# grantjr1842/delayed-streams-modeling

Hardware: AMD Instinct MI355X
Metric: real-time stream throughput, stt-1b-en_fr @ bs=64 per GPU (Mimi encode + LM decode per 80 ms frame) (higher is better)
Workload: dtype bf16 weights + bf16 KV, f32 activations as three exact bf16 pieces, f32 accumulate (v_mfma_f32_16x16x32_bf16); 1 GPU; stt-1b-en_fr batch=64 streaming, ring KV cache full (750 frames), Mimi encode + LM decode HIP path; streams_per_gpu=64, parallelism=replicas x1 (independent stream batches, no per-step collective), streams=encoder stream || 2 LM group stream(s)

## Files before the change

delayed-streams-modeling_amd/csrc/dsm_engine.hip:

```cpp
#include <hip/hip_runtime.h>

#include <cmath>
#include <cstdarg>
#include <cstdio>
#include <cstdlib>
#include <cstring>
#include <atomic>
#include <mutex>
#include <shared_mutex>
#include <string>
#include <set>
#include <vector>

#include "../../include/dsm.h"
#include "dsm_config_presets.h"
#include "dsm_kernels.h"
#include "dsm_numerics.h"
#include "dsm_safetensors.h"

static thread_local std::string g_create_error;

#define HIPCHK_E(eng, expr)                                                                         \
  do {                                                                                              \
    hipError_t _e = (expr);                                                                         \
// ... 23 lines not shown
  bool replicate = false;
};

struct TLayerW {
  Linear in_proj, out_proj, ff_in, ff_out;
  float *n1w = nullptr, *n1b = nullptr, *n2w = nullptr, *n2b = nullptr, *ls1 = nullptr, *ls2 = nullptr;
  Linear ca_q, ca_kv, ca_out;
  float *ncw = nullptr, *ncb = nullptr;
};

struct TransformerW {
  dsm_transformer_config cfg{};
  int hidden = 0;
  std::vector<TLayerW> layers;
  float* inv_freq = nullptr;
  bool rope_pos_before = false;
  bool has_ca = false;
  int ca_norm_rms = 0;
};

struct CaState {
  std::vector<void*> k, v;
  uint32_t* last = nullptr;
  uint8_t* act = nullptr;
  float* att = nullptr;
  int smax = 0;
};

struct TransformerState {
  std::vector<void*> k, v;
  uint32_t *pos = nullptr, *idx = nullptr, *start_pos = nullptr, *widx = nullptr;
  float* rope_cs = nullptr;
};

struct RvqW {
  Linear input_proj, output_proj;
  int n_q = 0;
  std::vector<Linear> codebooks;
};

struct MimiW {
  dsm_mimi_config cfg{};
  ConvGeom init_conv, final_conv, downsample;
  struct Stage {
    ConvGeom ra, rb, down;
  };
  std::vector<Stage> stages;
  TransformerW tr;
  RvqW rvq_first, rvq_rest;
  struct DecStage {
    Linear up;
    float* up_bias = nullptr;
    int in_c = 0, out_c = 0, k = 0, stride = 0, T_in = 0;
    ConvGeom ra, rb;
  };
  bool has_decoder = false;
  ConvGeom dec_init, dec_final;
  std::vector<DecStage> dec_stages;
  TransformerW dec_tr;
  float* upsample_w = nullptr;
  const float** emb_ptrs = nullptr;
};

struct MimiState {
  float* pcm = nullptr;
  float* cat_init = nullptr;
  struct Stage {
    float *y = nullptr, *cat_ra = nullptr, *cat_rb = nullptr, *cat_down = nullptr;
  };
  std::vector<Stage> stages;
  float* cat_final = nullptr;
  float *x_tr = nullptr, *xn = nullptr, *q = nullptr, *att = nullptr, *ff = nullptr;
  float* cat_ds = nullptr;
  float* latent = nullptr;
  float *res_first = nullptr, *res_rest = nullptr, *pval = nullptr;
  uint32_t* pidx = nullptr;
  uint32_t* codes = nullptr;
  TransformerState tr;
  ConvStateDesc* descs = nullptr;
  std::vector<ConvStateDesc> h_descs;
  int ds_desc = -1;
  bool first_call = true;
  uint8_t* mask = nullptr;
};

struct MimiDecState {
  bool ready = false, first_call = true;
  uint32_t* codes = nullptr;
  uint8_t* mask = nullptr;
  uint8_t* started = nullptr;
  float *q_first = nullptr, *q_rest = nullptr, *emb = nullptr, *up_carry = nullptr;
  float *x_tr = nullptr, *xn = nullptr, *q = nullptr, *att = nullptr, *ff = nullptr;
  TransformerState tr;
  float* cat_init = nullptr;
  struct Stage {
    float *x = nullptr, *z = nullptr, *carry = nullptr, *y = nullptr, *cat_ra = nullptr, *cat_rb = nullptr;
  };
  std::vector<Stage> stages;
  float* cat_final = nullptr;
  float* pcm = nullptr;
  ConvStateDesc* descs = nullptr;
  std::vector<ConvStateDesc> h_descs;
};

struct LmW {
  uint16_t* text_emb = nullptr;
  uint16_t* audio_emb = nullptr;
  TransformerW tr;
  float* out_norm = nullptr;
  Linear text_linear, extra_heads;
};

struct LmState {
  float *x = nullptr, *xn = nullptr, *q = nullptr, *att = nullptr, *g = nullptr, *hidden = nullptr, *logits = nullptr,
        *eh = nullptr, *prs = nullptr;
  uint32_t *next_cb = nullptr, *text_token = nullptr, *text_out = nullptr, *codes_in = nullptr;
  uint8_t *first_step = nullptr, *mask = nullptr;
  uint32_t* rng_key = nullptr;
  unsigned long long* rng_pos = nullptr;
  uint8_t* gmask = nullptr;
  TransformerState tr;
  struct Group {
    int b0 = 0, nb = 0;
    TransformerState view;
  };
  std::vector<Group> groups;
};

struct HostItem {
  size_t step_idx = 0;
  std::vector<uint32_t> word_tokens;
  bool unended_word = false;
  double last_stop_time = 0.0;
};

}

struct dsm_engine {
  dsm_asr_config cfg{};
  int B = 0, device = 0;
  hipStream_t s_enc = nullptr, s_model = nullptr;
  static constexpr int kMaxGroups = 4;
  hipStream_t s_grp[kMaxGroups] = {nullptr, nullptr, nullptr, nullptr};
  hipEvent_t ev_fork = nullptr, ev_grp_in[kMaxGroups] = {}, ev_grp_done[kMaxGroups] = {}, ev_stagger[kMaxGroups] = {};
  bool grp_busy = false;
  bool use_graphs = true;
  bool fuse_qkv = true;
  bool stream_prio = false;
  bool fuse_front = false;
  int chunk_loop_min_tiles = 384;
  int loop_depth = 4;
  int smallk_min_tiles = 1024;
  int smallk_mt = 4;
  size_t attn_lds_pad = 60000;
  int dot_mode = 0;
  int prio_hi = 0;
  bool serialize_groups = false;
  hipEvent_t ev_codes_consumed = nullptr;
  bool codes_consumed_valid = false;
  hipEvent_t ev_join = nullptr, ev_a = nullptr, ev_b = nullptr, ev_c = nullptr, ev_d = nullptr;
  MimiW mimi_w;
  MimiState mimi[2];
  std::atomic<bool> mimi1_ready{false};
  std::mutex mimi1_mu;
  MimiDecState dec;
  float* h_pcm_out = nullptr;
  LmW lm_w;
  LmState lm;
  std::vector<void*> allocs;
  std::string err;
  float* h_pcm = nullptr;
  float* h_pcm1 = nullptr;
  uint8_t* h_mask = nullptr;
  uint32_t *h_codes = nullptr, *h_text = nullptr;
  float* h_prs = nullptr;
  std::vector<HostItem> items;
  size_t model_step_idx = 0;
  std::vector<dsm_asr_msg> msgs;
  std::vector<uint32_t> msg_tokens;
  dsm_metrics metrics{};
  static constexpr int kStreams = 1 + kMaxGroups;
  float* gemm_ws[kStreams] = {};
  size_t gemm_ws_cap[kStreams] = {};
  std::atomic<uint64_t> ws_gen{0};
  struct GraphSlot {
    hipGraphExec_t exec = nullptr;
    uint64_t key = 0, ws_gen = 0;
    int warm = 0;
    int failures = 0;
    bool disabled = false;
  };
  static constexpr int kMaxCaptureTries = 3;
  static thread_local bool capturing;
  bool capture_failed = false;
  GraphSlot g_enc[2], g_grp[kMaxGroups], g_dec, g_ttsg[kMaxGroups][2];
  std::atomic<uint64_t> graph_launches{0}, eager_bodies{0}, capture_failures{0};
  std::string capture_error;
  void note_capture_failure(const char* what, hipError_t he) {
    capture_failures += 1;
    std::lock_guard<std::mutex> lk(err_mu);
    if (capture_error.empty()) {
      capture_error = what;
      if (he != hipSuccess) { capture_error += ": "; capture_error += hipGetErrorString(he); }
    }
  }
  static constexpr int kPipe = 4;
  struct PipeSlot {
    float* h_pcm = nullptr;
    uint8_t* h_mask = nullptr;
    uint32_t* d_codes = nullptr;
    hipEvent_t ev_done = nullptr, ev_consumed = nullptr;
    bool in_flight = false;
  };
  PipeSlot pipe[kPipe];
  int pipe_next = 0;
  bool pipe_ready = false;
  std::mutex pipe_mu;
  std::shared_mutex api_mu;
  static thread_local std::shared_lock<std::shared_mutex>* api_held;
  unsigned prof_mask = 0;
  int tag_gemm[kStreams] = {DSM_PROF_OTHER, DSM_PROF_OTHER, DSM_PROF_OTHER, DSM_PROF_OTHER, DSM_PROF_OTHER};
  int tag_attn[kStreams] = {DSM_PROF_OTHER, DSM_PROF_OTHER, DSM_PROF_OTHER, DSM_PROF_OTHER, DSM_PROF_OTHER};
  std::mutex prof_mu, err_mu;
  int sid(hipStream_t st) const {
    if (st == s_enc) return 0;
    for (int g = 1; g < kMaxGroups; ++g)
      if (st == s_grp[g]) return 1 + g;
    return 1;
  }
  struct ProfRec {
    int tag;
    hipEvent_t a, b;
  };
  std::vector<ProfRec> prof_recs;
  std::vector<hipEvent_t> prof_pool;
  double prof_total_us[DSM_PROF_NTAGS] = {0};
  uint64_t prof_launches[DSM_PROF_NTAGS] = {0};

  static constexpr size_t kDevTsCap = 1 << 16;
  unsigned long long* dev_ts = nullptr;
  std::vector<int> dev_ts_tags;
  std::vector<int> dev_ts_info;
  bool timeline = false;
  unsigned long long* dev_ts_slot(int tag, int sid_ = 0, int kind = 0, int n = 1) {
    if (!dev_ts || !(prof_mask & (1u << tag))) return nullptr;
    std::lock_guard<std::mutex> lk(prof_mu);
    if (dev_ts_tags.size() + n > kDevTsCap) return nullptr;
    unsigned long long* p = dev_ts + 2 * dev_ts_tags.size();
    for (int i = 0; i < n; ++i) {
      dev_ts_tags.push_back(tag);
      dev_ts_info.push_back((sid_ << 8) | (kind + i));
    }
    return p;
  }

  hipEvent_t prof_event() {
    if (!prof_pool.empty()) {
      hipEvent_t ev = prof_pool.back();
      prof_pool.pop_back();
      return ev;
    }
    hipEvent_t ev = nullptr;
    (void)hipEventCreate(&ev);
    return ev;
  }
  int prof_begin(int tag, hipStream_t st) {
    if (!(prof_mask & (1u << tag))) return -1;
    std::lock_guard<std::mutex> lk(prof_mu);
    ProfRec r{tag, prof_event(), prof_event()};
    (void)hipEventRecord(r.a, st);
    prof_recs.push_back(r);
    return (int)prof_recs.size() - 1;
  }
  void prof_end(int h, hipStream_t st) {
    if (h < 0) return;
    std::lock_guard<std::mutex> lk(prof_mu);
    (void)hipEventRecord(prof_recs[h].b, st);
  }

  void set_error(const char* fmt, ...) {
    char buf[1024];
    va_list ap;
    va_start(ap, fmt);
    vsnprintf(buf, sizeof buf, fmt, ap);
    va_end(ap);
    std::lock_guard<std::mutex> lk(err_mu);
    err = buf;
  }

  template <typename T>
  int dalloc(T** out, size_t count, bool zero = true) {
    void* p = nullptr;
    size_t bytes = count * sizeof(T) + 256;
    HIPCHK_E(this, hipMalloc(&p, bytes));
    if (zero) {
      HIPCHK_E(this, hipMemset(p, 0, bytes));
      HIPCHK_E(this, hipStreamSynchronize(nullptr));
    }
    allocs.push_back(p);
    *out = reinterpret_cast<T*>(p);
    return 0;
  }
  template <typename T>
  int upload(T** out, const T* host, size_t count) {
    if (int rc = dalloc(out, count)) return rc;
    HIPCHK_E(this, hipMemcpy(*out, host, count * sizeof(T), hipMemcpyHostToDevice));
// ... 373 lines not shown
  if (cfg.quantizer_n_q > 1)
    if (int rc = load_rvq(e, ld, &m->rvq_rest, "quantizer.rvq_rest", cfg.quantizer_n_q - 1, cfg)) return rc;
  m->has_decoder = ld.has("decoder.model.0.conv.conv.weight") || ld.has("decoder.model.0.conv.conv.weight_v");
  if (!m->has_decoder) return 0;
  {
    int mult = 1 << cfg.n_ratios, idx = 0, T = m->final_conv.T_out;
    char p[128];
    snprintf(p, sizeof p, "decoder.model.%d", idx);
    if (int rc = load_conv(e, ld, &m->dec_init, p, cfg.dimension, mult * cfg.n_filters, cfg.kernel_size, 1, true, false)) return rc;
    m->dec_init.T_in = m->dec_init.T_out = T;
    idx += 1;
    m->dec_stages.resize(cfg.n_ratios);
    for (int i = 0; i < cfg.n_ratios; ++i) {
      const int ratio = cfg.ratios[i];
      MimiW::DecStage& st = m->dec_stages[i];
      st.in_c = mult * cfg.n_filters;
      st.out_c = st.in_c / 2;
      st.k = 2 * ratio;
      st.stride = ratio;
      st.T_in = T;
      snprintf(p, sizeof p, "decoder.model.%d.convtr.convtr", idx + 1);
      std::vector<float> w;
      if (ld.has("%s.weight", p)) {
        w = ld.get((int64_t)st.in_c * st.out_c * st.k, "%s.weight", p);
      } else {
        auto g = ld.get(st.in_c, "%s.weight_g", p);
        w = ld.get((int64_t)st.in_c * st.out_c * st.k, "%s.weight_v", p);
        for (int ci = 0; ci < st.in_c && !ld.failed; ++ci) {
          float ss = 0.0f;
          const size_t n = (size_t)st.out_c * st.k;
          for (size_t j = 0; j < n; ++j) ss = ss + w[ci * n + j] * w[ci * n + j];
          float nrm = sqrtf(ss);
          for (size_t j = 0; j < n; ++j) w[ci * n + j] = w[ci * n + j] * g[ci] / nrm;
        }
      }
      auto b = ld.get(st.out_c, "%s.bias", p);
      if (ld.failed) return DSM_ERR_IO;
      std::vector<float> r((size_t)st.k * st.out_c * st.in_c);
      for (int ci = 0; ci < st.in_c; ++ci)
        for (int co = 0; co < st.out_c; ++co)
          for (int kk = 0; kk < st.k; ++kk)
            r[((size_t)kk * st.out_c + co) * st.in_c + ci] = w[((size_t)ci * st.out_c + co) * st.k + kk];
      if (int rc = pack_linear(e, &st.up, r.data(), st.k * st.out_c, st.in_c, false, nullptr)) return rc;
      if (int rc = e->upload_w(&st.up_bias, b.data(), b.size())) return rc;
      idx += 2;
      T *= ratio;
      const int dim = st.out_c, hidden = dim / cfg.compress;
      snprintf(p, sizeof p, "decoder.model.%d.block.1", idx);
      if (int rc = load_conv(e, ld, &st.ra, p, dim, hidden, cfg.residual_kernel_size, 1, true, false)) return rc;
      snprintf(p, sizeof p, "decoder.model.%d.block.3", idx);
      if (int rc = load_conv(e, ld, &st.rb, p, hidden, dim, 1, 1, true, false)) return rc;
      st.ra.T_in = st.ra.T_out = st.rb.T_in = st.rb.T_out = T;
      idx += 1;
      mult /= 2;
    }
    snprintf(p, sizeof p, "decoder.model.%d", idx + 1);
    if (int rc = load_conv(e, ld, &m->dec_final, p, cfg.n_filters, cfg.channels, cfg.last_kernel_size, 1, true, false)) return rc;
    m->dec_final.T_in = m->dec_final.T_out = T;
    if (T != DSM_FRAME_SIZE) {
      e->set_error("decoder emits %d samples per step, expected %d", T, DSM_FRAME_SIZE);
      return DSM_ERR_INVALID;
    }
    if (int rc = load_transformer(e, ld, &m->dec_tr, cfg.transformer, "decoder_transformer.transformer", false)) return rc;
    const int st_ = cfg.downsample_stride, dim = cfg.dimension;
    auto uw = ld.get((int64_t)dim * 2 * st_, "upsample.convtr.convtr.convtr.weight");
    if (ld.failed) return DSM_ERR_IO;
    std::vector<float> ur((size_t)2 * st_ * dim);
    for (int c = 0; c < dim; ++c)
      for (int kk = 0; kk < 2 * st_; ++kk) ur[(size_t)kk * dim + c] = uw[(size_t)c * 2 * st_ + kk];
    if (int rc = e->upload_w(&m->upsample_w, ur.data(), ur.size())) return rc;
    std::vector<const float*> ptrs;
    ptrs.push_back(reinterpret_cast<const float*>(m->rvq_first.codebooks[0].w));
    for (auto& cb : m->rvq_rest.codebooks) ptrs.push_back(reinterpret_cast<const float*>(cb.w));
    if (e->wmode != dsm_engine::W_MEASURE)
      if (int rc = e->upload(&m->emb_ptrs, ptrs.data(), ptrs.size())) return rc;
  }
  return 0;
}

int alloc_cat(dsm_engine* e, float** out, const ConvGeom& c, int B) {
  return e->dalloc(out, (size_t)B * (c.S + c.T_in) * c.in_c);
}

void add_desc(MimiState* s, float* cat, const ConvGeom& c) {
  if (c.S == 0) return;
  ConvStateDesc d;
  d.cat = cat;
  d.bstride = (long)(c.S + c.T_in) * c.in_c;
  d.S = c.S;
  d.T = c.T_in;
  d.C = c.in_c;
  d.replicate = c.replicate ? 1 : 0;
  s->h_descs.push_back(d);
}

int alloc_mimi_state(dsm_engine* e, MimiState* s, const MimiW& w, int B) {
  const dsm_mimi_config& cfg = w.cfg;
  if (int rc = alloc_cat(e, &s->cat_init, w.init_conv, B)) return rc;
  add_desc(s, s->cat_init, w.init_conv);
  s->stages.resize(w.stages.size());
  for (size_t i = 0; i < w.stages.size(); ++i) {
    const MimiW::Stage& st = w.stages[i];
    if (int rc = e->dalloc(&s->stages[i].y, (size_t)B * st.ra.T_in * st.ra.in_c)) return rc;
    if (int rc = alloc_cat(e, &s->stages[i].cat_ra, st.ra, B)) return rc;
    if (int rc = alloc_cat(e, &s->stages[i].cat_rb, st.rb, B)) return rc;
    if (int rc = alloc_cat(e, &s->stages[i].cat_down, st.down, B)) return rc;
    add_desc(s, s->stages[i].cat_ra, st.ra);
    add_desc(s, s->stages[i].cat_rb, st.rb);
    add_desc(s, s->stages[i].cat_down, st.down);
  }
  if (int rc = alloc_cat(e, &s->cat_final, w.final_conv, B)) return rc;
  add_desc(s, s->cat_final, w.final_conv);
  const int Tt = w.final_conv.T_out, d = cfg.dimension;
  if (int rc = e->dalloc(&s->x_tr, (size_t)B * Tt * d)) return rc;
  if (int rc = e->dalloc(&s->xn, (size_t)B * Tt * d)) return rc;
  if (int rc = e->dalloc(&s->q, (size_t)B * Tt * d)) return rc;
  if (int rc = e->dalloc(&s->att, (size_t)B * Tt * d)) return rc;
  if (int rc = e->dalloc(&s->ff, (size_t)B * Tt * cfg.transformer.dim_feedforward)) return rc;
  if (int rc = alloc_cat(e, &s->cat_ds, w.downsample, B)) return rc;
  s->ds_desc = (int)s->h_descs.size();
  add_desc(s, s->cat_ds, w.downsample);
  if (int rc = e->dalloc(&s->latent, (size_t)B * d)) return rc;
  if (int rc = e->dalloc(&s->res_first, (size_t)B * cfg.quantizer_dim)) return rc;
  if (int rc = e->dalloc(&s->res_rest, (size_t)B * cfg.quantizer_dim)) return rc;
  const int n_tiles = (cfg.quantizer_bins + 15) / 16;
  if (int rc = e->dalloc(&s->pval, (size_t)n_tiles * B)) return rc;
  if (int rc = e->dalloc(&s->pidx, (size_t)n_tiles * B)) return rc;
  if (int rc = e->dalloc(&s->codes, (size_t)B * cfg.quantizer_n_q)) return rc;
  if (int rc = e->dalloc(&s->mask, B)) return rc;
  if (int rc = alloc_transformer_state(e, &s->tr, cfg.transformer, B, Tt, false)) return rc;
  if (int rc = e->upload(&s->descs, s->h_descs.data(), s->h_descs.size())) return rc;
  s->pcm = s->cat_init + (size_t)w.init_conv.S * w.init_conv.in_c;
  return 0;
}

bool wk_applicable(const dsm_engine* e, bool bf16_weights, int Kpad, int K, int M) {
  const int chunks = (Kpad + DSM_KC - 1) / DSM_KC;
  return bf16_weights && e->dot_mode == 1 && K % 32 == 0 && Kpad == K && chunks <= 4 && M <= 64;
}

template <typename WT, typename KVT, int EPI, int NT, int MT>
void launch_tile(hipStream_t st, dim3 grid, const GemmArgs& a, bool bx3, bool roll, bool deep) {
  constexpr int DMAX = LoopDepth<WT, NT>::MAX;
  if (bx3 && EPI != EPI_RVQ) {
    if (a.chunk_loop > 1) hipLaunchKernelGGL((gemm_bx3_kernel<KVT, MT, NT, EPI, true>), grid, dim3(256), 0, st, a);
    else if constexpr (MT == 4) hipLaunchKernelGGL((gemm_bx3_kernel<KVT, 4, NT, EPI, false>), grid, dim3(256), 0, st, a);
    else if constexpr (MT == 2) hipLaunchKernelGGL((gemm_bx3u_kernel<KVT, 2, NT, EPI, 8, 0, 4>), grid, dim3(256), 8 * 3 * 32 * 32 * 2, st, a);
    else hipLaunchKernelGGL((gemm_bx3u_kernel<KVT, 1, NT, EPI, 8>), grid, dim3(256), 8 * 3 * 16 * 32 * 2, st, a);
  } else if (roll && deep) hipLaunchKernelGGL((gemm_loop_kernel<WT, KVT, MT, NT, EPI, DMAX>), grid, dim3(256), 0, st, a);
  else if (roll) hipLaunchKernelGGL((gemm_loop_kernel<WT, KVT, MT, NT, EPI, 2>), grid, dim3(256), 0, st, a);
  else hipLaunchKernelGGL((gemm_tile_kernel<WT, KVT, MT, NT, EPI>), grid, dim3(256), 0, st, a);
}

template <typename WT, typename KVT, int EPI, int NT>
int launch_gemm_tiled(dsm_engine* e, hipStream_t st, GemmArgs& a) {
  int chunks = (a.Kpad + DSM_KC - 1) / DSM_KC;
  const int gx = (a.N + 63) / 64;
  const bool bx3 = e->dot_mode == 1 && sizeof(WT) == 2;
  auto ok4 = [](const RowMap& m) { return m.ld % 4 == 0 && m.bstride % 4 == 0; };
  a.vec = (a.N % 4 == 0) && (!a.Y || ok4(a.ymap)) && (!a.Y2 || ok4(a.y2map)) && (!a.res || ok4(a.rmap));
  a.chunk_loop = 0;
  if (chunks > 1 && (long)gx * ((a.M + 63) / 64) >= e->chunk_loop_min_tiles) {
    a.chunk_loop = chunks;
    a.defer_reduce = 0;
    chunks = 1;
  }
  if constexpr (EPI == EPI_GATE && NT == 2) {
    if (wk_applicable(e, sizeof(WT) == 2, a.Kpad, a.K, a.M) && chunks > 1 && a.N % 16 == 0) {
      a.ts = e->timeline ? e->dev_ts_slot(e->tag_gemm[e->sid(st)], e->sid(st), 1, 2) : nullptr;
      const int ph = e->prof_begin(e->tag_gemm[e->sid(st)], st);
      hipLaunchKernelGGL((gemm_wk_kernel<KVT, 1, 2, EPI_GATE, 1, 4, 2, true, 4>), dim3(a.N / 16, 1, (a.M + 15) / 16), dim3(256),
                         (size_t)chunks * 2 * 1024, st, a);
      e->prof_end(ph, st);
      HIPCHK(hipGetLastError());
      return 0;
    }
  }
  int MT = a.M > 32 ? 4 : (a.M > 16 ? 2 : 1);
  while (MT > 1 && (long)gx * chunks * ((a.M + 16 * MT - 1) / (16 * MT)) < 256) MT /= 2;
  if (MT == 4 && bx3 && chunks > 1 && a.M <= 64 && (long)gx * chunks <= 256 && EPI == EPI_STORE) MT = 2;
  const bool smallk = chunks == 1 && a.chunk_loop == 0 && (long)gx * ((a.M + 63) / 64) >= e->smallk_min_tiles && !bx3;
  if (smallk && e->smallk_mt < MT) MT = e->smallk_mt;
  a.ws_ntiles = (((NT - 1) * a.nt_stride) >> 4) + gx * 4;
  const int mtiles = (a.M + 15) / 16;
  if (chunks > 1) {
    const int wsid = e->sid(st);
    size_t need = (size_t)chunks * mtiles * a.ws_ntiles * 256 * sizeof(float);
    if (need > e->gemm_ws_cap[wsid]) {
      if (e->capturing) {
        e->capture_failed = true;
        e->set_error("split-K workspace grew during a graph capture");
        return DSM_ERR_STATE;
      }
      e->ws_gen += 1;
      HIPCHK(hipStreamSynchronize(st));
      if (e->gemm_ws[wsid]) HIPCHK(hipFree(e->gemm_ws[wsid]));
      e->gemm_ws[wsid] = nullptr;
      e->gemm_ws_cap[wsid] = 0;
      void* p = nullptr;
      HIPCHK(hipMalloc(&p, need));
      e->gemm_ws[wsid] = reinterpret_cast<float*>(p);
      e->gemm_ws_cap[wsid] = need;
    }
    a.ws = e->gemm_ws[wsid];
  }
  dim3 grid(gx, chunks, (a.M + 16 * MT - 1) / (16 * MT));
  const bool nt2 = NT == 1 && bx3 && a.chunk_loop > 1 && MT == 4 && (EPI == EPI_STORE || EPI == EPI_QKV) && a.N % 128 == 0 &&
                   (long)(a.N / 128) * grid.z >= 256;
  if (nt2) {
    grid.x = a.N / 128;
    a.wg_cols = 128;
    a.nt_stride = 64;
  }
  a.ts = e->timeline ? e->dev_ts_slot(e->tag_gemm[e->sid(st)], e->sid(st), 1, 2) : nullptr;
  const int ph = e->prof_begin(e->tag_gemm[e->sid(st)], st);
  const bool roll = a.chunk_loop > 1 || smallk;
  const bool deep = LoopDepth<WT, NT>::MAX == 4 && e->loop_depth == 4 && !smallk;
  if (nt2) hipLaunchKernelGGL((gemm_bx3_kernel<KVT, 4, (NT == 1 ? 2 : NT), (EPI == EPI_GATE ? EPI_STORE : EPI), true>), grid, dim3(256), 0, st, a);
  else if (MT == 4) launch_tile<WT, KVT, EPI, NT, 4>(st, grid, a, bx3, roll, deep);
  else if (MT == 2) launch_tile<WT, KVT, EPI, NT, 2>(st, grid, a, bx3, roll, deep);
  else launch_tile<WT, KVT, EPI, NT, 1>(st, grid, a, bx3, roll, deep);
  const bool rows_ok = (EPI == EPI_STORE) && a.norm_out && a.vec && !a.Y2 && a.Y && a.N <= 4096 && a.ymap.bstride == 0;
  if (chunks > 1 && !((EPI == EPI_QKV || EPI == EPI_STORE) && a.defer_reduce)) {
    if (rows_ok) {
      if (a.N <= 1024) hipLaunchKernelGGL(gemm_reduce_rows_kernel<1>, dim3(a.M), dim3(256), 0, st, a, chunks);
      else if (a.N <= 2048) hipLaunchKernelGGL(gemm_reduce_rows_kernel<2>, dim3(a.M), dim3(512), 0, st, a, chunks);
      else hipLaunchKernelGGL(gemm_reduce_rows_kernel<4>, dim3(a.M), dim3(1024), 0, st, a, chunks);
    } else {
      const int out_tiles = mtiles * ((a.N + 15) / 16);
      hipLaunchKernelGGL((gemm_reduce_kernel<KVT, EPI>), dim3((out_tiles + 3) / 4), dim3(256), 0, st, a, chunks);
    }
  }
  e->prof_end(ph, st);
  HIPCHK(hipGetLastError());
  if (a.norm_out && !(chunks > 1 && rows_ok)) {
    hipLaunchKernelGGL(row_norm_kernel, dim3(a.M), dim3(256), 0, st, a.norm_out, a.Y, a.norm_w, a.norm_b, a.M,
                       a.N, a.norm_eps, a.norm_rms);
    HIPCHK(hipGetLastError());
  }
  return 0;
}

template <typename WT, typename KVT, int EPI, int NT>
int launch_gemm_t(dsm_engine* e, hipStream_t st, GemmArgs& a, bool aligned) {
  if (aligned && a.K % 32 == 0) return launch_gemm_tiled<WT, KVT, EPI, NT>(e, st, a);
  const int chunks = (a.Kpad + DSM_KC - 1) / DSM_KC;
  const int rounds = (chunks + 15) / 16;
  const int S = (chunks + rounds - 1) / rounds;
  const int tiles16 = (a.N + 15) / 16;
  const int nx = (EPI == EPI_GATE) ? tiles16 : (tiles16 + NT - 1) / NT;
  int MT = (NT == 2) ? 2 : 4;
  while (MT > 1 && (a.M <= 16 * (MT / 2) || (long)nx * ((a.M + 16 * MT - 1) / (16 * MT)) * S < 2048 ||
                    (chunks > 1 && (size_t)chunks * NT * MT * 1024 > 64 * 1024)))
    MT /= 2;
  if (chunks > 1 && (size_t)chunks * NT * MT * 1024 > 160 * 1024) {
    e->set_error("GEMM K=%d: chunk partials do not fit in LDS", a.K);
    return DSM_ERR_INVALID;
  }
  auto ok4 = [](const RowMap& m) { return m.ld % 4 == 0 && m.bstride % 4 == 0; };
  a.vec = (a.N % 4 == 0) && (!a.Y || ok4(a.ymap)) && (!a.Y2 || ok4(a.y2map)) && (!a.res || ok4(a.rmap));
  aligned = aligned && (a.K % 32 == 0);
  dim3 grid(nx, (a.M + 16 * MT - 1) / (16 * MT));
  dim3 block(64 * S);
  size_t lds = chunks > 1 ? (size_t)chunks * NT * MT * 1024 : 0;
  const bool bx3 = e->dot_mode == 1 && sizeof(WT) == 2 && EPI != EPI_RVQ;
#define DSM_LAUNCH(MTv, AL)                                                                                   \
  do {                                                                                                        \
    if (bx3) hipLaunchKernelGGL((gemm_mfma_kernel<WT, KVT, MTv, NT, EPI, AL, true>), grid, block, lds, st, a); \
    else hipLaunchKernelGGL((gemm_mfma_kernel<WT, KVT, MTv, NT, EPI, AL>), grid, block, lds, st, a);          \
  } while (0)
  const int ph = e->prof_begin(e->tag_gemm[e->sid(st)], st);
  if (MT == 1) {
    if (aligned) DSM_LAUNCH(1, true); else DSM_LAUNCH(1, false);
  } else if (MT == 2) {
    if (aligned) DSM_LAUNCH(2, true); else DSM_LAUNCH(2, false);
  } else {
    if (aligned) DSM_LAUNCH(4, true); else DSM_LAUNCH(4, false);
  }
  e->prof_end(ph, st);
#undef DSM_LAUNCH
  HIPCHK(hipGetLastError());
  if (a.norm_out) {
    hipLaunchKernelGGL(row_norm_kernel, dim3(a.M), dim3(256), 0, st, a.norm_out, a.Y, a.norm_w, a.norm_b, a.M,
                       a.N, a.norm_eps, a.norm_rms);
    HIPCHK(hipGetLastError());
  }
  return 0;
}

template <typename F>
int run_captured(dsm_engine* e, dsm_engine::GraphSlot& gs, hipStream_t st, uint64_t key, F&& body) {
  if (!e->use_graphs || e->prof_mask != 0 || gs.disabled) { e->eager_bodies += 1; return body(); }
  if (gs.exec && gs.key == key && gs.ws_gen == e->ws_gen) {
    HIPCHK(hipGraphLaunch(gs.exec, st));
    e->graph_launches += 1;
    return 0;
  }
  if (gs.key != key || gs.ws_gen != e->ws_gen) {
    gs.key = key;
    gs.ws_gen = e->ws_gen;
    gs.warm = 0;
    if (gs.exec) { (void)hipGraphExecDestroy(gs.exec); gs.exec = nullptr; }
  }
  if (gs.warm < 2) {
    gs.warm += 1;
    e->eager_bodies += 1;
    const int rc = body();
    if (gs.ws_gen != e->ws_gen) { gs.ws_gen = e->ws_gen; gs.warm = 0; }
    return rc;
  }
  ApiExclusive alone(e);
  hipError_t hb = hipStreamBeginCapture(st, hipStreamCaptureModeRelaxed);
  if (hb != hipSuccess) {
    (void)hipGetLastError();
    e->note_capture_failure("hipStreamBeginCapture", hb);
    if (++gs.failures >= dsm_engine::kMaxCaptureTries) gs.disabled = true;
    gs.warm = 0;
    e->eager_bodies += 1;
// ... 86 lines not shown
```

delayed-streams-modeling_amd/csrc/dsm_engine_api.inc:

```

namespace {

template <typename KVT, int HD, int T>
int launch_attn_t(dsm_engine* e, hipStream_t st, float* out, const float* q, const void* k, const void* v,
                  const uint32_t* start_pos, const uint8_t* active, int B, int H, int ctx, int d, const AttnFused& fq) {
  constexpr int UNR = (sizeof(KVT) == 2 && T == 1 && HD == 128) ? 8 : 4;
  size_t lds = sizeof(float) * ((size_t)T * ctx + 4 * T * HD + 16);
  if ((long)B * H >= 2048 && (size_t)2 * ctx * HD * sizeof(KVT) >= (size_t)256 * 1024) lds += e->attn_lds_pad;
  if (lds > 64 * 1024) {
    static size_t allowed = 0;
    if (lds > allowed) {
      HIPCHK(hipFuncSetAttribute(reinterpret_cast<const void*>(&attn_kernel<KVT, HD, T, UNR>), hipFuncAttributeMaxDynamicSharedMemorySize, (int)lds));
      allowed = lds;
    }
  }
  const int tag = e->tag_attn[e->sid(st)];
  if (T == 1 && HD == 64 && ctx <= 32) {
    const int ph = e->prof_begin(tag, st);
    hipLaunchKernelGGL((attn_small_kernel<KVT, 64>), dim3((B * H + 3) / 4), dim3(256), 0, st, out, q, reinterpret_cast<const KVT*>(k),
                       reinterpret_cast<const KVT*>(v), start_pos, active, B * H, H, ctx, d, fq);
    e->prof_end(ph, st);
    HIPCHK(hipGetLastError());
    return 0;
  }
// ... 1372 lines not shown
}

int dsm_prof_read(dsm_engine* e, double* total_us, uint64_t* launches) {
  if (!e) return DSM_ERR_INVALID;
  ApiShared api(e);
  if (int rc = dsm_sync(e)) return rc;
  for (auto& r : e->prof_recs) {
    float ms = 0;
    if (hipEventElapsedTime(&ms, r.a, r.b) == hipSuccess) {
      e->prof_total_us[r.tag] += ms * 1000.0;
      e->prof_launches[r.tag] += 1;
    }
    e->prof_pool.push_back(r.a);
    e->prof_pool.push_back(r.b);
  }
  e->prof_recs.clear();
  for (int i = 0; i < DSM_PROF_NTAGS; ++i) {
    if (total_us) total_us[i] = e->prof_total_us[i];
    if (launches) launches[i] = e->prof_launches[i];
    e->prof_total_us[i] = 0;
    e->prof_launches[i] = 0;
  }
  return 0;
}

int dsm_lm_stream_groups(dsm_engine* e, int* first_slot, int* n_slots, int cap) {
  if (!e) return DSM_ERR_INVALID;
  const int G = (int)e->lm.groups.size();
  for (int g = 0; g < G && g < cap; ++g) {
    if (first_slot) first_slot[g] = e->lm.groups[g].b0;
    if (n_slots) n_slots[g] = e->lm.groups[g].nb;
  }
  return G;
}

int dsm_debug_serialize_groups(dsm_engine* e, int on) {
  if (!e) return DSM_ERR_INVALID;
  HIPCHK(hipSetDevice(e->device));
  ApiShared api(e);
  if (int rc = dsm_sync(e)) return rc;
  e->serialize_groups = on != 0;
  return 0;
}

int dsm_prof_read_device(dsm_engine* e, double* total_us, uint64_t* launches) {
  if (!e) return DSM_ERR_INVALID;
  HIPCHK(hipSetDevice(e->device));
  ApiShared api(e);
  if (int rc = dsm_sync(e)) return rc;
  for (int i = 0; i < DSM_PROF_NTAGS; ++i) {
    if (total_us) total_us[i] = 0;
    if (launches) launches[i] = 0;
  }
  const size_t n = e->dev_ts_tags.size();
  if (n) {
    std::vector<unsigned long long> h(2 * n);
    HIPCHK(hipMemcpy(h.data(), e->dev_ts, sizeof(unsigned long long) * 2 * n, hipMemcpyDeviceToHost));
    int khz = 100000;
    (void)hipDeviceGetAttribute(&khz, hipDeviceAttributeWallClockRate, e->device);
    for (size_t i = 0; i < n; ++i) {
      if (h[2 * i + 1] < h[2 * i]) continue;
      if (total_us) total_us[e->dev_ts_tags[i]] += (double)(h[2 * i + 1] - h[2 * i]) * 1000.0 / khz;
      if (launches) launches[e->dev_ts_tags[i]] += 1;
    }
    for (size_t i = 0; i < n; ++i) { h[2 * i] = ~0ull; h[2 * i + 1] = 0; }
    HIPCHK(hipMemcpy(e->dev_ts, h.data(), sizeof(unsigned long long) * 2 * n, hipMemcpyHostToDevice));
    HIPCHK(hipStreamSynchronize(nullptr));
  }
  e->dev_ts_tags.clear();
  e->dev_ts_info.clear();
  return 0;
}

int dsm_prof_timeline(dsm_engine* e, int on) {
  if (!e) return DSM_ERR_INVALID;
  e->timeline = on != 0;
  return 0;
}

int dsm_prof_timeline_read(dsm_engine* e, int* sid, int* kind, int* tag, double* start_us, double* end_us, int cap) {
  if (!e) return DSM_ERR_INVALID;
  HIPCHK(hipSetDevice(e->device));
  ApiShared api(e);
  if (int rc = dsm_sync(e)) return rc;
  const size_t n = e->dev_ts_tags.size();
  int out = 0;
  if (n) {
    std::vector<unsigned long long> h(2 * n);
    HIPCHK(hipMemcpy(h.data(), e->dev_ts, sizeof(unsigned long long) * 2 * n, hipMemcpyDeviceToHost));
    int khz = 100000;
    (void)hipDeviceGetAttribute(&khz, hipDeviceAttributeWallClockRate, e->device);
    unsigned long long t0 = ~0ull;
    for (size_t i = 0; i < n; ++i)
      if (h[2 * i + 1] >= h[2 * i] && h[2 * i] < t0) t0 = h[2 * i];
    for (size_t i = 0; i < n && out < cap; ++i) {
      if (h[2 * i + 1] < h[2 * i]) continue;
      sid[out] = e->dev_ts_info[i] >> 8;
      kind[out] = e->dev_ts_info[i] & 0xff;
      tag[out] = e->dev_ts_tags[i];
      start_us[out] = (double)(h[2 * i] - t0) * 1000.0 / khz;
      end_us[out] = (double)(h[2 * i + 1] - t0) * 1000.0 / khz;
      ++out;
    }
    for (size_t i = 0; i < n; ++i) { h[2 * i] = ~0ull; h[2 * i + 1] = 0; }
    HIPCHK(hipMemcpy(e->dev_ts, h.data(), sizeof(unsigned long long) * 2 * n, hipMemcpyHostToDevice));
    HIPCHK(hipStreamSynchronize(nullptr));
  }
  e->dev_ts_tags.clear();
  e->dev_ts_info.clear();
  return out;
}

int dsm_debug_set_positions(dsm_engine* e, uint32_t lm_pos, uint32_t mimi_pos) {
  if (!e) return DSM_ERR_INVALID;
  HIPCHK(hipSetDevice(e->device));
  ApiShared api(e);
  if (int rc = dsm_sync(e)) return rc;
  auto fill = [&](TransformerState& s, uint32_t pos, int ctx) {
    unsigned g = (unsigned)((e->B + 255) / 256);
    hipLaunchKernelGGL(fill_u32_kernel, dim3(g), dim3(256), 0, e->s_model, s.pos, pos, (long)e->B);
    hipLaunchKernelGGL(fill_u32_kernel, dim3(g), dim3(256), 0, e->s_model, s.idx, pos % (uint32_t)ctx, (long)e->B);
  };
  fill(e->lm.tr, lm_pos, e->cfg.lm.context);
  for (int side = 0; side < 2; ++side)
    if (side == 0 || e->mimi1_ready.load(std::memory_order_acquire)) fill(e->mimi[side].tr, mimi_pos, e->cfg.mimi.transformer.context);
  HIPCHK(hipGetLastError());
  return dsm_sync(e);
}

int dsm_debug_set_text_tokens(dsm_engine* e, const uint32_t* tokens) {
  if (!e || !tokens) return DSM_ERR_INVALID;
  HIPCHK(hipSetDevice(e->device));
  ApiShared api(e);
  if (int rc = dsm_sync(e)) return rc;
  HIPCHK(hipMemcpy(e->lm.text_token, tokens, sizeof(uint32_t) * (size_t)e->B, hipMemcpyHostToDevice));
  return dsm_sync(e);
}

int dsm_debug_read(dsm_engine* e, const char* name, float* out, size_t cap) {
  if (!e || !name || !out) return DSM_ERR_INVALID;
  HIPCHK(hipSetDevice(e->device));
  ApiShared api(e);
  if (int rc = dsm_sync(e)) return rc;
  const float* src = nullptr;
  size_t n = 0;
  const int B = e->B, dim = e->cfg.mimi.dimension;
  int side = 0;
  std::string nm(name);
  if (nm.rfind("mimi1.", 0) == 0) { side = 1; nm = nm.substr(6); }
  else if (nm.rfind("mimi.", 0) == 0) nm = nm.substr(5);
  if (nm == "lm.hidden") { src = e->lm.hidden; n = (size_t)B * e->cfg.lm.d_model; }
  else if (nm == "lm.logits") { src = e->lm.logits; n = (size_t)B * e->cfg.text_out_vocab_size; }
  else if (nm == "latent") { src = e->mimi[side].latent; n = (size_t)B * dim; }
  if (!src) { e->set_error("unknown debug tap %s", name); return DSM_ERR_INVALID; }
  if (n > cap) n = cap;
  HIPCHK(hipMemcpy(out, src, sizeof(float) * n, hipMemcpyDeviceToHost));
  return (int)n;
}

}
```

delayed-streams-modeling_amd/csrc/dsm_kernels.h:

```cpp
#pragma once
#include <hip/hip_runtime.h>
#include <stdint.h>
#include "dsm_numerics.h"
#include "dsm_sampling.h"

typedef float f32x4 __attribute__((ext_vector_type(4)));
typedef short dsm_bf16x8 __attribute__((ext_vector_type(8)));

__device__ __forceinline__ float wave_sum64(float v) {
#pragma unroll
  for (int off = 32; off >= 1; off >>= 1) v = v + __shfl_xor(v, off, 64);
  return v;
}

enum { EPI_STORE = 0, EPI_QKV = 1, EPI_GATE = 2, EPI_RVQ = 3 };

struct RowMap {
  long bstride;
  int rpb;
  int ld;
  int toff;
  __host__ __device__ long off(int m) const { return (long)(m / rpb) * bstride + (long)((m % rpb) + toff) * ld; }
};

// ... 484 lines not shown
    return;
  }
#pragma unroll
  for (int mt = 0; mt < MT; ++mt) {
    const int m = m_base + 16 * mt + r;
    if (EPI == EPI_GATE) {
      epi_gate(a, acc[0][mt], acc[NT - 1][mt], m, n_base + 4 * q);
    } else {
#pragma unroll
      for (int nt = 0; nt < NT; ++nt) {
        const int n = n_base + nt * a.nt_stride + 4 * q;
        if (EPI == EPI_RVQ)
          epi_rvq(a, acc[nt][mt], m, n, (n_base + nt * a.nt_stride) >> 4, q);
        else
          epi_store_qkv<KVT, EPI>(a, acc[nt][mt], m, n);
      }
    }
  }
  launch_stamp_end(a.ts);
}

template <typename WT, int NT>
struct LoopDepth {
  static constexpr int MAX = (NT == 2 || sizeof(WT) == 4) ? 2 : 4;
};
template <typename WT, typename KVT, int MT, int NT, int EPI, int D, int OCC = 2>
__global__ __launch_bounds__(256, OCC) void gemm_loop_kernel(GemmArgs a) {
  static_assert(D == 2 || D == 4, "window depth");
  launch_stamp_begin(a.ts);
  __shared__ __attribute__((aligned(16))) float Xs[2][16 * MT][DSM_XS_LD];
  const int tid = threadIdx.x, lane = tid & 63, wave = tid >> 6;
  const int r = lane & 15, q = lane >> 4;
  const int xu0 = 4 * ((2 * q) ^ dsm_xs_sw(r)), xu1 = xu0 ^ 4;
  const int m_base = blockIdx.z * (16 * MT);
  const int n_base = blockIdx.x * 64 + 16 * wave;
  const WT* W = reinterpret_cast<const WT*>(a.W);
  const WT* wrow[NT];
#pragma unroll
  for (int nt = 0; nt < NT; ++nt) wrow[nt] = dsm_wbase<WT>(a, W, n_base + nt * a.nt_stride, r, q);
  const int wst = dsm_wstep<WT>(a);
  constexpr int PIECES = 16 * MT * 8;
  constexpr bool TWO = PIECES > 256;
  const bool has0 = tid < PIECES;
  const int row0 = has0 ? (tid >> 3) : 0, part = tid & 7;
  int m0 = m_base + row0;
  m0 = m0 < a.M ? m0 : a.M - 1;
  const float* xsrc0 = a.X + a.xmap.off(m0) + 4 * part;
  const int xdst0 = row0 * DSM_XS_LD + 4 * (part ^ dsm_xs_sw(row0));
  int m1 = m_base + row0 + 32;
  m1 = m1 < a.M ? m1 : a.M - 1;
  const float* xsrc1 = a.X + a.xmap.off(m1) + 4 * part;
  const int xdst1 = (row0 + 32) * DSM_XS_LD + 4 * (part ^ dsm_xs_sw(row0));
  const int nb = a.Kpad >> 5;

  f32x4 acc[NT][MT], tot[NT][MT];
#pragma unroll
  for (int nt = 0; nt < NT; ++nt)
#pragma unroll
    for (int mt = 0; mt < MT; ++mt) {
      acc[nt][mt] = (f32x4){0.f, 0.f, 0.f, 0.f};
      tot[nt][mt] = (f32x4){0.f, 0.f, 0.f, 0.f};
    }
  float4 xp0, xp1, xp2, xp3, xq0, xq1, xq2, xq3;
  Raw8<WT> rw0[NT], rw1[NT], rw2[NT], rw3[NT];
#define DSM_LLOAD(S, G)                                                              \
  {                                                                                  \
    const int kb_ = 32 * min((G), nb - 1);                                           \
    xp##S = *reinterpret_cast<const float4*>(xsrc0 + kb_);                           \
    xq##S = TWO ? *reinterpret_cast<const float4*>(xsrc1 + kb_) : xp##S;             \
    _Pragma("unroll") for (int nt = 0; nt < NT; ++nt) rw##S[nt].load(wrow[nt] + (long)kb_ * wst); \
  }
  DSM_LLOAD(0, 0) DSM_LLOAD(1, 1)
  if (D == 4) { DSM_LLOAD(2, 2) DSM_LLOAD(3, 3) }
  __builtin_amdgcn_sched_barrier(0);
  float xbA[MT][8], xbB[MT][8];
#define DSM_LSTORE(S, BUF)                                                           \
  {                                                                                  \
    float* xs_ = &Xs[BUF][0][0];                                                     \
    if (has0) *reinterpret_cast<float4*>(xs_ + xdst0) = xp##S;                       \
    if (TWO) *reinterpret_cast<float4*>(xs_ + xdst1) = xq##S;                        \
  }
#define DSM_LFRAG(XB, BUF)                                                           \
  _Pragma("unroll") for (int mt = 0; mt < MT; ++mt) {                                \
    const float* fp = &Xs[BUF][0][0] + (16 * mt + r) * DSM_XS_LD;                    \
    const float4 f0 = *reinterpret_cast<const float4*>(fp + xu0), f1 = *reinterpret_cast<const float4*>(fp + xu1); \
    XB[mt][0] = f0.x; XB[mt][1] = f0.y; XB[mt][2] = f0.z; XB[mt][3] = f0.w;          \
    XB[mt][4] = f1.x; XB[mt][5] = f1.y; XB[mt][6] = f1.z; XB[mt][7] = f1.w;          \
  }
  DSM_LSTORE(0, 0)
  __syncthreads();
  DSM_LFRAG(xbA, 0)
#define DSM_LMFMA(CUR, S0, S1)                                                       \
  _Pragma("unroll") for (int s = (S0); s < (S1); ++s) {                              \
    _Pragma("unroll") for (int nt = 0; nt < NT; ++nt)                                \
    _Pragma("unroll") for (int mt = 0; mt < MT; ++mt)                                \
      acc[nt][mt] = __builtin_amdgcn_mfma_f32_16x16x4f32(wa[nt][s], CUR[mt][s], acc[nt][mt], 0, 0, 0); \
    if (NT * MT > 1) __builtin_amdgcn_sched_barrier(0);  \
  }
#define DSM_LSTEP(S, SN, CUR, NXT)                                                   \
  {                                                                                  \
    const int gb = g + (S);                                                          \
    float wa[NT][8];                                                                 \
    _Pragma("unroll") for (int nt = 0; nt < NT; ++nt) rw##S[nt].unpack(wa[nt]);      \
    if (gb < nb) {                                            \
      if (gb + 1 < nb) DSM_LSTORE(SN, ((S) + 1) & 1)                                 \
      __syncthreads();                                                               \
       \
      DSM_LMFMA(CUR, 0, 1)                                                           \
      if (gb + 1 < nb) { DSM_LFRAG(NXT, ((S) + 1) & 1) }                             \
      __builtin_amdgcn_sched_barrier(0);                                             \
    }                                                                                \
    DSM_LLOAD(S, gb + D)  \
    __builtin_amdgcn_sched_barrier(0);                                               \
    if (gb < nb) {                                                                   \
      DSM_LMFMA(CUR, 1, 8)                                                           \
      if ((gb & 7) == 7 || gb == nb - 1) {  \
        _Pragma("unroll") for (int nt = 0; nt < NT; ++nt)                            \
        _Pragma("unroll") for (int mt = 0; mt < MT; ++mt) {                          \
          tot[nt][mt] = tot[nt][mt] + acc[nt][mt];  \
          acc[nt][mt] = (f32x4){0.f, 0.f, 0.f, 0.f};                                 \
        }                                                                            \
      }                                                                              \
    }                                                                                \
  }
#pragma clang loop unroll(disable)
  for (int g = 0; g < nb; g += D) {
    if (D == 4) {
      DSM_LSTEP(0, 1, xbA, xbB) DSM_LSTEP(1, 2, xbB, xbA) DSM_LSTEP(2, 3, xbA, xbB) DSM_LSTEP(3, 0, xbB, xbA)
    } else {
      DSM_LSTEP(0, 1, xbA, xbB) DSM_LSTEP(1, 0, xbB, xbA)
    }
  }
#undef DSM_LSTORE
#undef DSM_LFRAG
#undef DSM_LMFMA
#undef DSM_LLOAD
#undef DSM_LSTEP
#pragma unroll
  for (int mt = 0; mt < MT; ++mt) {
    const int m = m_base + 16 * mt + r;
    if (EPI == EPI_GATE) {
      epi_gate(a, tot[0][mt], tot[NT - 1][mt], m, n_base + 4 * q);
    } else {
#pragma unroll
      for (int nt = 0; nt < NT; ++nt) {
        const int n = n_base + nt * a.nt_stride + 4 * q;
        if (EPI == EPI_RVQ)
          epi_rvq(a, tot[nt][mt], m, n, (n_base + nt * a.nt_stride) >> 4, q);
        else
          epi_store_qkv<KVT, EPI>(a, tot[nt][mt], m, n);
      }
    }
  }
  launch_stamp_end(a.ts);
}

template <typename KVT, int MT, int NT, int EPI, bool LOOP>
__global__ __launch_bounds__(256, 2) void gemm_bx3_kernel(GemmArgs a) {
  __shared__ __attribute__((aligned(16))) uint16_t Xp[2][3][16 * MT][32];
  launch_stamp_begin(a.ts);
  const int tid = threadIdx.x, lane = tid & 63, wave = tid >> 6;
  const int r = lane & 15, q = lane >> 4;
  const int chunks = LOOP ? 1 : (int)gridDim.y;
  const int m_base = blockIdx.z * (16 * MT);
  const int n_base = blockIdx.x * (a.wg_cols ? a.wg_cols : 64) + 16 * wave;
  const uint16_t* W = reinterpret_cast<const uint16_t*>(a.W);
  const uint16_t* wrow[NT];
#pragma unroll
  for (int nt = 0; nt < NT; ++nt) wrow[nt] = dsm_wbase<uint16_t>(a, W, n_base + nt * a.nt_stride, r, q);
  const int wst = dsm_wstep<uint16_t>(a);
  constexpr int PIECES = 16 * MT * 8;
  constexpr bool TWO = PIECES > 256;
  const bool has0 = tid < PIECES;
  const int row0 = has0 ? (tid >> 3) : 0, part = tid & 7;
  int m0 = m_base + row0;
  m0 = m0 < a.M ? m0 : a.M - 1;
  const float* xsrc0 = a.X + a.xmap.off(m0) + 4 * part;
  int m1 = m_base + row0 + 32;
  m1 = m1 < a.M ? m1 : a.M - 1;
  const float* xsrc1 = a.X + a.xmap.off(m1) + 4 * part;
  auto stage = [&](int buf, const float4& v, int row) {
    uint16_t h[4], m[4], l[4];
    dsm_split3(v.x, &h[0], &m[0], &l[0]); dsm_split3(v.y, &h[1], &m[1], &l[1]);
    dsm_split3(v.z, &h[2], &m[2], &l[2]); dsm_split3(v.w, &h[3], &m[3], &l[3]);
    const int off = row * 32 + (((part >> 1) ^ ((row >> 1) & 3)) * 8) + (part & 1) * 4;
    *reinterpret_cast<uint2*>(&Xp[buf][0][0][0] + off) = make_uint2((uint32_t)l[0] | ((uint32_t)l[1] << 16), (uint32_t)l[2] | ((uint32_t)l[3] << 16));
    *reinterpret_cast<uint2*>(&Xp[buf][1][0][0] + off) = make_uint2((uint32_t)m[0] | ((uint32_t)m[1] << 16), (uint32_t)m[2] | ((uint32_t)m[3] << 16));
    *reinterpret_cast<uint2*>(&Xp[buf][2][0][0] + off) = make_uint2((uint32_t)h[0] | ((uint32_t)h[1] << 16), (uint32_t)h[2] | ((uint32_t)h[3] << 16));
  };
  const int kb0 = LOOP ? 0 : (int)blockIdx.y * (DSM_KC >> 5);
  const int kb1 = LOOP ? (a.Kpad >> 5) : min(kb0 + (DSM_KC >> 5), a.Kpad >> 5);
  f32x4 acc[NT][MT], tot[NT][MT];
#pragma unroll
  for (int nt = 0; nt < NT; ++nt)
#pragma unroll
    for (int mt = 0; mt < MT; ++mt) {
      acc[nt][mt] = (f32x4){0.f, 0.f, 0.f, 0.f};
      tot[nt][mt] = (f32x4){0.f, 0.f, 0.f, 0.f};
    }
  float4 xa = *reinterpret_cast<const float4*>(xsrc0 + 32 * kb0);
  float4 xb = TWO ? *reinterpret_cast<const float4*>(xsrc1 + 32 * kb0) : xa;
  uint4 wv[NT];
#pragma unroll
  for (int nt = 0; nt < NT; ++nt) wv[nt] = *reinterpret_cast<const uint4*>(wrow[nt] + (long)32 * kb0 * wst);
  for (int g = kb0; g < kb1; ++g) {
    const int buf = (g - kb0) & 1;
    if (has0) stage(buf, xa, row0);
    if (TWO) stage(buf, xb, row0 + 32);
    dsm_bf16x8 wa[NT];
#pragma unroll
    for (int nt = 0; nt < NT; ++nt) {
      const uint4 w = wv[nt];
      wa[nt][0] = (short)(w.x & 0xFFFF); wa[nt][1] = (short)(w.x >> 16); wa[nt][2] = (short)(w.y & 0xFFFF); wa[nt][3] = (short)(w.y >> 16);
      wa[nt][4] = (short)(w.z & 0xFFFF); wa[nt][5] = (short)(w.z >> 16); wa[nt][6] = (short)(w.w & 0xFFFF); wa[nt][7] = (short)(w.w >> 16);
    }
    {
      const int gn = g + 1 < kb1 ? g + 1 : g;
      xa = *reinterpret_cast<const float4*>(xsrc0 + 32 * gn);
      if (TWO) xb = *reinterpret_cast<const float4*>(xsrc1 + 32 * gn);
#pragma unroll
      for (int nt = 0; nt < NT; ++nt) wv[nt] = *reinterpret_cast<const uint4*>(wrow[nt] + (long)32 * gn * wst);
    }
    __syncthreads();
#pragma unroll
    for (int p = 0; p < 3; ++p)
#pragma unroll
      for (int mt = 0; mt < MT; ++mt) {
        const int row = 16 * mt + r;
        const dsm_bf16x8 xf = *reinterpret_cast<const dsm_bf16x8*>(&Xp[buf][p][0][0] + row * 32 + ((q ^ ((row >> 1) & 3)) * 8));
#pragma unroll
        for (int nt = 0; nt < NT; ++nt) acc[nt][mt] = __builtin_amdgcn_mfma_f32_16x16x32_bf16(wa[nt], xf, acc[nt][mt], 0, 0, 0);
      }
    if (LOOP && ((g & 7) == 7 || g == kb1 - 1)) {
#pragma unroll
      for (int nt = 0; nt < NT; ++nt)
#pragma unroll
        for (int mt = 0; mt < MT; ++mt) {
          tot[nt][mt] = tot[nt][mt] + acc[nt][mt];
          acc[nt][mt] = (f32x4){0.f, 0.f, 0.f, 0.f};
        }
    }
  }
  if (!LOOP) {
#pragma unroll
    for (int nt = 0; nt < NT; ++nt)
#pragma unroll
      for (int mt = 0; mt < MT; ++mt) tot[nt][mt] = (f32x4){0.f, 0.f, 0.f, 0.f} + acc[nt][mt];
  }
  if (chunks > 1) {
    const long ld = (long)a.ws_ntiles * 16;
    const long mpad = (long)((a.M + 15) >> 4) * 16;
#pragma unroll
    for (int mt = 0; mt < MT; ++mt) {
      const int m = m_base + 16 * mt + r;
      if (m >= mpad) continue;
#pragma unroll
      for (int nt = 0; nt < NT; ++nt) {
        const int n = n_base + nt * a.nt_stride + 4 * q;
        *reinterpret_cast<f32x4*>(a.ws + ((long)blockIdx.y * mpad + m) * ld + n) = tot[nt][mt];
      }
    }
    launch_stamp_end(a.ts);
    return;
  }
#pragma unroll
  for (int mt = 0; mt < MT; ++mt) {
    const int m = m_base + 16 * mt + r;
    if (EPI == EPI_GATE) {
      epi_gate(a, tot[0][mt], tot[NT - 1][mt], m, n_base + 4 * q);
    } else {
#pragma unroll
      for (int nt = 0; nt < NT; ++nt) epi_store_qkv<KVT, EPI>(a, tot[nt][mt], m, n_base + nt * a.nt_stride + 4 * q);
    }
  }
  launch_stamp_end(a.ts);
}

__device__ __forceinline__ f32x4 slab_sum(const float* p, long cstride, int chunks) {
  f32x4 t = *reinterpret_cast<const f32x4*>(p);
  for (int c0 = 1; c0 < chunks; c0 += 8) {
    f32x4 v[8];
#pragma unroll
    for (int u = 0; u < 8; ++u) {
      const int c = c0 + u < chunks ? c0 + u : chunks - 1;
      v[u] = *reinterpret_cast<const f32x4*>(p + c * cstride);
    }
#pragma unroll
    for (int u = 0; u < 8; ++u)
      if (c0 + u < chunks) t = t + v[u];
  }
  return t;
}

template <typename KVT, int EPI>
__global__ __launch_bounds__(256) void gemm_reduce_kernel(GemmArgs a, int chunks) {
  launch_stamp_begin(a.ts ? a.ts + 2 : nullptr);
  const int lane = threadIdx.x & 63, wave = threadIdx.x >> 6;
  const int r = lane & 15, q = lane >> 4;
  const int mtiles = (a.M + 15) >> 4;
  const int out_ntiles = (a.N + 15) >> 4;
  const int t = blockIdx.x * 4 + wave;
  if (t >= mtiles * out_ntiles) return;
  const int mtile = t / out_ntiles, ntile = t % out_ntiles;
  constexpr int NT = (EPI == EPI_GATE) ? 2 : 1;
  const long ld = (long)a.ws_ntiles * 16, cstride = (long)mtiles * 16 * ld;
  const int m = mtile * 16 + r, n = ntile * 16 + 4 * q;
// ... 1268 lines not shown
```

Before: 1821 x realtime (stream-seconds of audio per wall second).

## Route f32-weight chunk-looped conv GEMMs to a dedicated fp32 MFMA register-tiled kernel

Adds a conv_gemm_kernel that computes f32-weight, store-epilogue GEMMs with large K (chunk_loop) and N<=512 using v_mfma_f32_16x16x4f32. It uses a multi-tile register blocking of MT x NT, double-buffered global loads and periodic partial-sum flushes. Tile shape is picked from three forms to minimise wave-slot cost, and a separate row-norm kernel runs when norm_out is set. The goal is to speed up the Mimi encoder's f32 convolution GEMMs compared with the generic tile/loop kernels. The trade-offs are a second launch for the norm and loads that skip LDS, which could cost bandwidth reuse. A launch counter exposed through a debug tap is also added.

```diff
diff --git a/delayed-streams-modeling_amd/csrc/dsm_engine.hip b/delayed-streams-modeling_amd/csrc/dsm_engine.hip
--- a/delayed-streams-modeling_amd/csrc/dsm_engine.hip
+++ b/delayed-streams-modeling_amd/csrc/dsm_engine.hip
@@ -199,6 +199,7 @@
   int loop_depth = 4;
   int smallk_min_tiles = 1024;
   int smallk_mt = 4;
+  std::atomic<long> conv_gemm_launches{0};
   size_t attn_lds_pad = 60000;
   int dot_mode = 0;
   int prio_hi = 0;
@@ -878,6 +879,41 @@
   else hipLaunchKernelGGL((gemm_tile_kernel<WT, KVT, MT, NT, EPI>), grid, dim3(256), 0, st, a);
 }
 
+template <typename KVT>
+int launch_conv_gemm(dsm_engine* e, hipStream_t st, GemmArgs& a) {
+  static const int forms[3][2] = {{4, 4}, {2, 4}, {2, 2}};
+  int MT = 4, NT = 4;
+  long best = -1;
+  for (const auto& f : forms) {
+    const long tiles = (long)((a.M + 16 * f[0] - 1) / (16 * f[0])) * ((a.N + 16 * f[1] - 1) / (16 * f[1]));
+    const long cost = ((tiles + 1023) / 1024) * f[0] * f[1];
+    if (best < 0 || cost < best) {
+      best = cost;
+      MT = f[0];
+      NT = f[1];
+    }
+  }
+  const int ncol = (a.N + 16 * NT - 1) / (16 * NT);
+  const int wc = ncol >= 4 ? 4 : (ncol >= 2 ? 2 : 1);
+  a.wg_cols = wc * 16 * NT;
+  const int mtiles = (a.M + 16 * MT - 1) / (16 * MT);
+  dim3 grid((ncol + wc - 1) / wc, 1, (mtiles + 4 / wc - 1) / (4 / wc));
+  a.ts = e->timeline ? e->dev_ts_slot(e->tag_gemm[e->sid(st)], e->sid(st), 1, 2) : nullptr;
+  const int ph = e->prof_begin(e->tag_gemm[e->sid(st)], st);
+  if (MT == 4) hipLaunchKernelGGL((conv_gemm_kernel<KVT, 4, 4>), grid, dim3(256), 0, st, a);
+  else if (NT == 4) hipLaunchKernelGGL((conv_gemm_kernel<KVT, 2, 4>), grid, dim3(256), 0, st, a);
+  else hipLaunchKernelGGL((conv_gemm_kernel<KVT, 2, 2>), grid, dim3(256), 0, st, a);
+  e->prof_end(ph, st);
+  e->conv_gemm_launches.fetch_add(1, std::memory_order_relaxed);
+  HIPCHK(hipGetLastError());
+  if (a.norm_out) {
+    hipLaunchKernelGGL(row_norm_kernel, dim3(a.M), dim3(256), 0, st, a.norm_out, a.Y, a.norm_w, a.norm_b, a.M, a.N, a.norm_eps,
+                       a.norm_rms);
+    HIPCHK(hipGetLastError());
+  }
+  return 0;
+}
+
 template <typename WT, typename KVT, int EPI, int NT>
 int launch_gemm_tiled(dsm_engine* e, hipStream_t st, GemmArgs& a) {
   int chunks = (a.Kpad + DSM_KC - 1) / DSM_KC;
@@ -890,6 +926,9 @@
     a.chunk_loop = chunks;
     a.defer_reduce = 0;
     chunks = 1;
+  }
+  if constexpr (sizeof(WT) == 4 && EPI == EPI_STORE && NT == 1) {
+    if (a.chunk_loop > 1 && a.N <= 512) return launch_conv_gemm<KVT>(e, st, a);
   }
   if constexpr (EPI == EPI_GATE && NT == 2) {
     if (wk_applicable(e, sizeof(WT) == 2, a.Kpad, a.K, a.M) && chunks > 1 && a.N % 16 == 0) {
diff --git a/delayed-streams-modeling_amd/csrc/dsm_engine_api.inc b/delayed-streams-modeling_amd/csrc/dsm_engine_api.inc
--- a/delayed-streams-modeling_amd/csrc/dsm_engine_api.inc
+++ b/delayed-streams-modeling_amd/csrc/dsm_engine_api.inc
@@ -1548,6 +1548,11 @@
   if (nm == "lm.hidden") { src = e->lm.hidden; n = (size_t)B * e->cfg.lm.d_model; }
   else if (nm == "lm.logits") { src = e->lm.logits; n = (size_t)B * e->cfg.text_out_vocab_size; }
   else if (nm == "latent") { src = e->mimi[side].latent; n = (size_t)B * dim; }
+  else if (nm == "conv_gemm_launches") {
+    if (cap < 1) return 0;
+    out[0] = (float)e->conv_gemm_launches.load(std::memory_order_relaxed);
+    return 1;
+  }
   if (!src) { e->set_error("unknown debug tap %s", name); return DSM_ERR_INVALID; }
   if (n > cap) n = cap;
   HIPCHK(hipMemcpy(out, src, sizeof(float) * n, hipMemcpyDeviceToHost));
diff --git a/delayed-streams-modeling_amd/csrc/dsm_kernels.h b/delayed-streams-modeling_amd/csrc/dsm_kernels.h
--- a/delayed-streams-modeling_amd/csrc/dsm_kernels.h
+++ b/delayed-streams-modeling_amd/csrc/dsm_kernels.h
@@ -660,6 +660,86 @@
       }
     }
   }
+  launch_stamp_end(a.ts);
+}
+
+template <typename KVT, int MT, int NT>
+__global__ __launch_bounds__(256) void conv_gemm_kernel(GemmArgs a) {
+  launch_stamp_begin(a.ts);
+  const int lane = threadIdx.x & 63, wave = threadIdx.x >> 6;
+  const int r = lane & 15, q = lane >> 4;
+  const int wc = a.wg_cols / (16 * NT);
+  const int m_base = ((int)blockIdx.z * (4 / wc) + wave / wc) * (16 * MT);
+  const int n_base = ((int)blockIdx.x * wc + wave % wc) * (16 * NT);
+  const int nb = a.Kpad >> 5;
+  const int wtiles = (a.N + 15) >> 4;
+  const float* wp[NT];
+  const float* xp[MT];
+#pragma unroll
+  for (int nt = 0; nt < NT; ++nt) {
+    int t = (n_base >> 4) + nt;
+    t = t < wtiles ? t : wtiles - 1;
+    wp[nt] = reinterpret_cast<const float*>(a.W) + (long)(16 * t + r) * a.Kpad + 8 * q;
+  }
+#pragma unroll
+  for (int mt = 0; mt < MT; ++mt) {
+    int m = m_base + 16 * mt + r;
+    m = m < a.M ? m : a.M - 1;
+    xp[mt] = a.X + a.xmap.off(m) + 8 * q;
+  }
+  f32x4 acc[NT][MT], tot[NT][MT];
+#pragma unroll
+  for (int nt = 0; nt < NT; ++nt)
+#pragma unroll
+    for (int mt = 0; mt < MT; ++mt) {
+      acc[nt][mt] = (f32x4){0.f, 0.f, 0.f, 0.f};
+      tot[nt][mt] = (f32x4){0.f, 0.f, 0.f, 0.f};
+    }
+  f32x4 xa[MT][2], wa[NT][2], xb[MT][2], wb[NT][2];
+#define DSM_CLOAD(XF, WF, G)                                                          \
+  {                                                                                   \
+    const int kb_ = 32 * min((G), nb - 1);                                            \
+    _Pragma("unroll") for (int nt = 0; nt < NT; ++nt) {                               \
+      WF[nt][0] = *reinterpret_cast<const f32x4*>(wp[nt] + kb_);                      \
+      WF[nt][1] = *reinterpret_cast<const f32x4*>(wp[nt] + kb_ + 4);                  \
+    }                                                                                 \
+    _Pragma("unroll") for (int mt = 0; mt < MT; ++mt) {                               \
+      XF[mt][0] = *reinterpret_cast<const f32x4*>(xp[mt] + kb_);                      \
+      XF[mt][1] = *reinterpret_cast<const f32x4*>(xp[mt] + kb_ + 4);                  \
+    }                                                                                 \
+    __builtin_amdgcn_sched_barrier(0);                                                \
+  }
+#define DSM_CMFMA(XF, WF, GB)                                                         \
+  {                                                                                   \
+    _Pragma("unroll") for (int s = 0; s < 8; ++s) {                                   \
+      _Pragma("unroll") for (int nt = 0; nt < NT; ++nt)                               \
+      _Pragma("unroll") for (int mt = 0; mt < MT; ++mt)                               \
+        acc[nt][mt] = __builtin_amdgcn_mfma_f32_16x16x4f32(WF[nt][s >> 2][s & 3], XF[mt][s >> 2][s & 3], acc[nt][mt], 0, 0, 0); \
+      __builtin_amdgcn_sched_barrier(0);       \
+    }                                                                                 \
+    if ((((GB) & 7) == 7) || (GB) == nb - 1) {  \
+      _Pragma("unroll") for (int nt = 0; nt < NT; ++nt)                               \
+      _Pragma("unroll") for (int mt = 0; mt < MT; ++mt) {                             \
+        tot[nt][mt] = tot[nt][mt] + acc[nt][mt];  \
+        acc[nt][mt] = (f32x4){0.f, 0.f, 0.f, 0.f};                                    \
+      }                                                                               \
+    }                                                                                 \
+  }
+  DSM_CLOAD(xa, wa, 0)
+#pragma clang loop unroll(disable)
+  for (int g = 0; g < nb; g += 2) {
+    DSM_CLOAD(xb, wb, g + 1)
+    DSM_CMFMA(xa, wa, g)
+    DSM_CLOAD(xa, wa, g + 2)
+    if (g + 1 < nb) DSM_CMFMA(xb, wb, g + 1)
+  }
+#undef DSM_CLOAD
+#undef DSM_CMFMA
+#pragma unroll
+  for (int mt = 0; mt < MT; ++mt)
+#pragma unroll
+    for (int nt = 0; nt < NT; ++nt)
+      epi_store_qkv<KVT, EPI_STORE>(a, tot[nt][mt], m_base + 16 * mt + r, n_base + 16 * nt + 4 * q);
   launch_stamp_end(a.ts);
 }
 
```

Result: slower. 1734 x realtime (stream-seconds of audio per wall second) (-4.8%).
